# aehogan/lammps-induced-dipole-polarization-pair-style

Hardware: AMD Instinct MI355X
Metric: atom-steps/sec (higher is better)
Workload: dtype f64

## Files before the change

### lammps-induced-dipole-polarization-pair-style_amd/csrc/lab/api_env_knobs.inc

```
  if (const char *e = getenv("POLAR_ABLATE")) h->ablate = atoi(e);
  if (const char *e = getenv("POLAR_HOST_COLORS")) h->host_colors = atoi(e) != 0;
  if (const char *e = getenv("POLAR_SWEEP_KERNEL")) h->sweep_kernel = atoi(e);
  if (const char *e = getenv("POLAR_TILE_WAVES")) h->tile_waves = atoi(e) == 8 ? 8 : 4;
  if (const char *e = getenv("POLAR_TILE_WIDE")) h->tile_wide = atoi(e) != 0;
  if (const char *e = getenv("POLAR_CACHE_R2")) h->cache_r2 = atoi(e);
  if (const char *e = getenv("POLAR_LJ_TYPED")) h->lj_typed = atoi(e) != 0;
  if (const char *e = getenv("POLAR_STATIC_XQ")) h->static_xq = atoi(e) != 0;
  if (const char *e = getenv("POLAR_POL_FIRST")) h->pol_first = atoi(e) != 0;
  if (const char *e = getenv("POLAR_LP_WG_PER_CU")) h->lp_wg_per_cu = atoi(e);
  if (const char *e = getenv("POLAR_LP_QM")) h->lp_quad_major = atoi(e) != 0;
  if (const char *e = getenv("POLAR_LP_TILES")) h->lp_tiles = atoi(e) == 1 ? 1 : 2;
  if (const char *e = getenv("POLAR_LP_ROWS")) h->lp_rows = std::max(1, std::min(64, atoi(e)));
  if (const char *e = getenv("POLAR_LP_PAIRS")) h->lp_pairs = atoi(e) != 0;
  if (const char *e = getenv("POLAR_CLUSTER_DIST")) h->cluster_dist = atof(e);
  if (const char *e = getenv("POLAR_CLUSTER_MAX")) h->cluster_max = std::max(1, std::min(4, atoi(e)));
  if (const char *e = getenv("POLAR_LP_DEPTH")) { int v = atoi(e); h->lp_depth = (v == 2 || v == 3) ? v : 0; }
  if (const char *e = getenv("POLAR_QUAD_BLOCK")) { int v = atoi(e); if (v >= 64 && v <= 1024 && v % 64 == 0) h->quad_block = v; }
  if (const char *e = getenv("POLAR_FIELD_BLOCK")) { int v = atoi(e); if (v >= 64 && v <= 1024 && v % 64 == 0) h->field_block = v; }
```

### lammps-induced-dipole-polarization-pair-style_amd/csrc/polar_common.hpp

```cpp
#pragma once

#include <hip/hip_runtime.h>
#include <stdint.h>

#ifdef POLAR_LAB
#define POLAR_LAB_PARAM , int ablate
#define POLAR_LAB_PASS , ablate
#define POLAR_ABL(bit) (ablate & (bit))
#else
#define POLAR_LAB_PARAM
#define POLAR_LAB_PASS
#define POLAR_ABL(bit) 0
#endif

namespace polar {


struct __attribute__((aligned(64))) AtomRec {
  double x, mx;
  double y, my;
  double z, mz;
  double q, a;
};

// ... 227 lines not shown
  const double2 p0 = *reinterpret_cast<const double2 *>(base + ((j0 << 5) + piece));
  const double2 p1 = *reinterpret_cast<const double2 *>(base + ((j1 << 5) + piece));
  stage[h2 * 3 + k] = p0; stage[(32 + h2) * 3 + k] = p1;
  __builtin_amdgcn_fence(__ATOMIC_RELEASE, "wavefront");
  __builtin_amdgcn_wave_barrier();
  __builtin_amdgcn_fence(__ATOMIC_ACQUIRE, "wavefront");
  XQ r;
  r.a = stage[lane * 3]; r.b = stage[lane * 3 + 1];
  __builtin_amdgcn_wave_barrier();
  return r;
}

struct ExpCoef {
  double log2e, ln2hi, ln2lo;
  double c[14];
};
inline ExpCoef make_expcoef() {
  ExpCoef K;
  K.log2e = 1.4426950408889634074; K.ln2hi = 6.93147180369123816490e-01; K.ln2lo = 1.90821492927058770002e-10;
  const double c[14] = {1.0, 1.0, 0.5, 0.16666666666666666, 0.041666666666666664, 0.008333333333333333, 0.001388888888888889, 0.0001984126984126984, 2.48015873015873e-05, 2.7557319223985893e-06, 2.755731922398589e-07, 2.505210838544172e-08, 2.08767569878681e-09, 1.6059043836821613e-10};
  for (int k = 0; k < 14; k++) K.c[k] = c[k];
  return K;
}
__device__ __forceinline__ double exp_neg(double x, const ExpCoef &K) {
  x = fmax(x, -745.0);
  const double n = rint(x * K.log2e);
  double r = fma(-n, K.ln2hi, x);
  r = fma(-n, K.ln2lo, r);
  double p = K.c[13];
#pragma unroll
  for (int k = 12; k >= 0; k--) p = fma(p, r, K.c[k]);
  return ldexp(p, (int)n);
}

template <int DAMP>
__device__ __forceinline__ void tensor_scalars(double r2, double pd, double &s3, double &s5) {
  double rinv = rsqrt(r2);
  double r = r2 * rinv;
  double rinv2 = rinv * rinv;
  double r3 = rinv * rinv2;
  double r5 = r3 * rinv2;
  if (DAMP == 0) {
    double ar = pd * r;
    double e = exp(-ar);
    double p2 = 1.0 + ar + 0.5 * ar * ar;
    double p3 = p2 + ar * ar * ar * (1.0 / 6.0);
    s3 = (1.0 - e * p2) * r3;
    s5 = 3.0 * (1.0 - e * p3) * r5;
  } else {
    s3 = r3;
    s5 = 3.0 * r5;
  }
}
template <int DAMP>
__device__ __forceinline__ void tensor_scalars_k(double r2, double pd, const ExpCoef &K, double &s3, double &s5) {
  double rinv = rsqrt(r2);
  double r = r2 * rinv;
  double rinv2 = rinv * rinv;
  double r3 = rinv * rinv2;
  double r5 = r3 * rinv2;
  if (DAMP == 0) {
    double ar = pd * r;
    double e = exp_neg(-ar, K);
    double p2 = 1.0 + ar + 0.5 * ar * ar;
    double p3 = p2 + ar * ar * ar * (1.0 / 6.0);
    s3 = (1.0 - e * p2) * r3;
// ... 22 lines not shown
```

### lammps-induced-dipole-polarization-pair-style_amd/csrc/polar_handle.hpp

```cpp
#pragma once
#include <hip/hip_runtime.h>

#include <algorithm>
#include <initializer_list>
#include <utility>
#include <chrono>
#include <cmath>
#include <cstdio>
#include <cstdlib>
#include <exception>
#include <cstring>
#include <numeric>
#include <string>
#include <thread>
#include <mutex>
#include <condition_variable>
#include <functional>
#include <memory>
#include <stdexcept>
#include <unistd.h>
#include <vector>

#include "pair_host.hpp"
#include "polar_kernels.hpp"
// ... 165 lines not shown
  long long slots_epoch = -1;
  bool colors_recheck = false;
  std::vector<int> h_color;
  DBuf<int> d_color_orig, d_color_s;
  DBuf<int> d_klist;
  DBuf<int> d_cadj, d_cdeg, d_ccnt, d_cflags, d_crelabel;
  DBuf<unsigned long long> d_cprio;
  DBuf<double> d_cstat;
  DBuf<long long> d_coff;
  int *h_cflags = nullptr;
  double *h_cstat = nullptr;
  long long *h_coff = nullptr;
  int cadj_pitch = 16;
  int host_colors = 0;
  int colors_reused = 0, colors_rebuilt = 0;
  double ms_color_host = 0.0;
  double color_dist = 2.4;
  int field_block = 256;
  double bbox_lo[3] = {0, 0, 0}, bbox_hi[3] = {0, 0, 0};
  long long global_count = 0;
  DBuf<double> d_xchg; DBuf<int> d_xidx;
  bool device_list = false;
  int user_full_list = 0;
  long long lj_pitch = 0;
  DBuf<double4> d_ljpos; DBuf<int2> d_ljaux; DBuf<int> d_tag, d_nspecial, d_special, d_ljcell_id, d_ljcell_cnt, d_ljcell_fill; DBuf<long long> d_ljcell_first; DBuf<double> d_cutneighsq;
  int lj_typed = 1;
  bool lj_tab_arith = false;
  int lj_pers = 1;
  int ncu = 0;
  int lj_pers_threads = 768;
  bool sym_typed = false, dev_typed = false;
  int static_xq = 1;
  int pol_first = 1;
  int part_k = 0, part_n = 1;
  int lp_wg_per_cu = 0;
  int lp_quad_major = 1;
  int quad_block = POLAR_BLOCK;
  int lp_tiles = 2;
  int lp_rows = 1;
  int lp_pairs = 0;
  DBuf<int> d_ulead, d_udd_j;
  DBuf<long long> d_upos;
  DBuf<int2> d_unit;
  DBuf<int4> d_udesc;
  std::vector<int> unit_off;
  long long upitch = 0;
  int lp_depth = 0;
  int cache_r2 = -1;
  int stream_mode = 1;
  int sweep_kernel = 2;
  int ablate = 0;
  DBuf<SRec> d_srec0, d_srec1;
  DBuf<TileHdr> d_thdr;
  DBuf<TileRowEnt> d_trow;
  DBuf<int> d_un_j;
  DBuf<unsigned short> d_dd16;
  DBuf<double> d_pend;
  int un_pitch = 0;
  int un_lds = 0;
  long long pitch16 = 0;
  int tile_max_u = 0;
  bool tile_reported = false;
  double dens = 0.0;
  std::vector<TileLaunch> tile_launches;
  TileLaunch tile_all{};
  size_t tile_lds_attr[16] = {0, 0, 0, 0, 0, 0, 0, 0, 0, 0, 0, 0, 0, 0, 0, 0};
// ... 216 lines not shown
```

### lammps-induced-dipole-polarization-pair-style_amd/csrc/polar_rows.hpp

```cpp
#pragma once

#include "polar_common.hpp"

namespace polar {

static __global__ void k_pack(int n, const int *__restrict__ perm, const double *__restrict__ x, const double *__restrict__ q,
                       const double *__restrict__ alpha, const int *__restrict__ mol, const double *__restrict__ mu0,
                       AtomRec *__restrict__ r0, AtomRec *__restrict__ r1, int *__restrict__ mol_s,
                       double4 *__restrict__ pos4, double4 *__restrict__ xq_s, int wrap, Box box, double lo0, double lo1,
                       double lo2) {
  int i = blockIdx.x * blockDim.x + threadIdx.x;
  if (i == n) {
    AtomRec d;
    d.x = n > 0 ? x[0] : 0.0; d.y = n > 0 ? x[1] : 0.0; d.z = n > 0 ? x[2] : 0.0;
    d.mx = d.my = d.mz = d.q = d.a = 0.0;
    r0[n] = d; r1[n] = d;
  }
  if (i >= n) return;
  const int o = perm ? perm[i] : i;
  AtomRec r;
  r.x = x[3 * o]; r.y = x[3 * o + 1]; r.z = x[3 * o + 2]; r.q = q[o];
  if (wrap) {
    const double lo[3] = {lo0, lo1, lo2};
    double fr[3];
    frac_coords(box, lo, r.x, r.y, r.z, fr);
    const double n2 = box.periodic[2] ? floor(fr[2]) : 0.0, n1 = box.periodic[1] ? floor(fr[1]) : 0.0,
                 n0 = box.periodic[0] ? floor(fr[0]) : 0.0;
    r.z -= n2 * box.prd[2]; r.y -= n2 * box.yz + n1 * box.prd[1]; r.x -= n2 * box.xz + n1 * box.xy + n0 * box.prd[0];
  }
  r.mx = mu0 ? mu0[3 * o] : 0.0; r.my = mu0 ? mu0[3 * o + 1] : 0.0; r.mz = mu0 ? mu0[3 * o + 2] : 0.0;
  r.a = alpha[o];
  r0[i] = r;
  r1[i] = r;
  mol_s[i] = mol[o];
  if (pos4) pos4[i] = make_double4(r.x, r.y, r.z, __hiloint2double(mol[o], r.a != 0.0 ? 1 : 0));
// ... 413 lines not shown
      mx *= gamma; my *= gamma; mz *= gamma;
      rec0[i].mx = mx; rec0[i].my = my; rec0[i].mz = mz;
      rec1[i].mx = mx; rec1[i].my = my; rec1[i].mz = mz;
    }
  }
}

template <bool ALLPAIRS>
static __global__ __launch_bounds__(POLAR_BLOCK) void k_static_field(const int *__restrict__ rows, int nrows, int nlocal,
                                                              const AtomRec *__restrict__ rec,
                                                              const int *__restrict__ mol, Box box,
                                                              RowList nl,
                                                              const int *__restrict__ nl_j, double cut_coulsq,
                                                              double e2s, double gamma, int use_previous,
                                                              double *__restrict__ ef, AtomRec *__restrict__ rec0,
                                                              AtomRec *__restrict__ rec1, const double4 *__restrict__ xq_s) {
  static_field_body<ALLPAIRS, false>(rows, nrows, nlocal, rec, mol, box, nl, nl_j, cut_coulsq, e2s, gamma, use_previous, ef, rec0, rec1,
                                     xq_s, 0.0, nullptr);
}
template <bool ALLPAIRS>
static __global__ __launch_bounds__(POLAR_BLOCK) void k_ew_static_field(const int *__restrict__ rows, int nrows, int nlocal,
                                                                 const AtomRec *__restrict__ rec,
                                                                 const int *__restrict__ mol, Box box,
                                                                 RowList nl,
                                                                 const int *__restrict__ nl_j, double cut_coulsq,
                                                                 double e2s, double gamma, int use_previous,
                                                                 double *__restrict__ ef, AtomRec *__restrict__ rec0,
                                                                 AtomRec *__restrict__ rec1, const double4 *__restrict__ xq_s,
                                                                 double g_ewald, const double *__restrict__ erec) {
  static_field_body<ALLPAIRS, true>(rows, nrows, nlocal, rec, mol, box, nl, nl_j, cut_coulsq, e2s, gamma, use_previous, ef, rec0, rec1,
                                    xq_s, g_ewald, erec);
}

template <bool ALLPAIRS, int DAMP, bool EFLAG, bool VPAIR, bool EW>
static __device__ __forceinline__ void polar_force_body(const int *__restrict__ rows, int nrows, const int *__restrict__ perm,
                                                             int nlocal, const Scal *scal_in,
                                                             const AtomRec *__restrict__ recA,
                                                             const AtomRec *__restrict__ recB,
                                                             const int *__restrict__ mol, Box box,
                                                             RowList nl,
                                                             const int *__restrict__ nl_j, double cut_coulsq,
                                                             double ddcutsq, double pd, double e2s,
                                                             double *__restrict__ f, double *__restrict__ slots,
                                                             double *__restrict__ vatom, int vglobal, ExpCoef K,
                                                             double *__restrict__ dbg6, double g_ewald) {
  const int lane = threadIdx.x & 63;
  const int row = blockIdx.x * POLAR_ROWS_PER_BLOCK + (threadIdx.x >> 6);
  if (row >= nrows) return;
  const int i = rows ? rows[row] : row;
  const AtomRec *__restrict__ rec = __builtin_amdgcn_readfirstlane(scal_in->cur) ? recB : recA;
  const AtomRec ri = uniform_rec(rec[i]);
  const int mi = mol[i];
  const double f_shift = -1.0 / cut_coulsq;
  double fx = 0, fy = 0, fz = 0, uef = 0, udd = 0;
  double v0 = 0, v1 = 0, v2 = 0, v3 = 0, v4 = 0, v5 = 0;
  const bool isdbg = dbg6 && (perm ? perm[i] : i) == 0;
  double ddx = 0, ddy = 0, ddz = 0;
  long long beg = 0, end = nlocal;
  if (!ALLPAIRS) row_range(nl, i, beg, end);
  for (long long p = beg + lane; p < end; p += 64) {
    const int e = ALLPAIRS ? (int)p : nl_j[p];
    const int j = ALLPAIRS ? e : (e & POLAR_NL_MASK);
    if (j == i) continue;
    const AtomRec rj = *reinterpret_cast<const AtomRec *>(reinterpret_cast<const char *>(rec) + ((unsigned)j << 6));
    const bool molok = ALLPAIRS ? ((mi != mol[j]) || mi == 0) : !(e & POLAR_NL_SAMEMOL);
    double dx, dy, dz;
    pair_del<ALLPAIRS>(box, ri.x, ri.y, ri.z, rj.x, rj.y, rj.z, dx, dy, dz);
    const double xsq = dx * dx, ysq = dy * dy, zsq = dz * dz;
    const double rsq = xsq + ysq + zsq;
    const double rinv = rsqrt(rsq);
    const double r2inv = rinv * rinv;
    const double r = rsq * rinv;
    const double r3inv = r2inv * rinv;
    double px = 0, py = 0, pz = 0;
    if (EW) {
      if (rsq <= cut_coulsq) {
        double b1, b2;
        ewald_b12(rsq, g_ewald, molok, b1, b2);
        if (ri.a != 0.0 && rj.q != 0.0) {
          const double c = rj.q * e2s, pr = (ri.mx * dx + ri.my * dy + ri.mz * dz) * b2;
          px += c * (b1 * ri.mx - pr * dx); py += c * (b1 * ri.my - pr * dy); pz += c * (b1 * ri.mz - pr * dz);
        }
        if (rj.a != 0.0 && ri.q != 0.0) {
          const double c = ri.q * e2s, pr = (rj.mx * dx + rj.my * dy + rj.mz * dz) * b2;
          px -= c * (b1 * rj.mx - pr * dx); py -= c * (b1 * rj.my - pr * dy); pz -= c * (b1 * rj.mz - pr * dz);
        }
      }
    } else if (rsq < cut_coulsq && molok) {
      const double mxx = (-2.0 * xsq + ysq + zsq) * r2inv + f_shift * (ysq + zsq);
      const double myy = (-2.0 * ysq + xsq + zsq) * r2inv + f_shift * (xsq + zsq);
      const double mzz = (-2.0 * zsq + xsq + ysq) * r2inv + f_shift * (xsq + ysq);
      const double k = -(3.0 * r2inv + f_shift);
      const double mxy = k * dx * dy, mxz = k * dx * dz, myz = k * dy * dz;
      const double ef_temp = (r2inv + f_shift) * rinv * e2s;
      if (ri.a != 0.0 && rj.q != 0.0) {
        const double cf = rj.q * e2s * r3inv;
        px += cf * (ri.mx * mxx + ri.my * mxy + ri.mz * mxz);
        py += cf * (ri.mx * mxy + ri.my * myy + ri.mz * myz);
        pz += cf * (ri.mx * mxz + ri.my * myz + ri.mz * mzz);
        if (EFLAG) uef -= ef_temp * rj.q * (ri.mx * dx + ri.my * dy + ri.mz * dz);
      }
      if (rj.a != 0.0 && ri.q != 0.0) {
        const double cf = ri.q * e2s * r3inv;
        px -= cf * (rj.mx * mxx + rj.my * mxy + rj.mz * mxz);
        py -= cf * (rj.mx * mxy + rj.my * myy + rj.mz * myz);
        pz -= cf * (rj.mx * mxz + rj.my * myz + rj.mz * mzz);
        if (EFLAG) uef += ef_temp * ri.q * (rj.mx * dx + rj.my * dy + rj.mz * dz);
      }
    }
    if (ri.a != 0.0 && rj.a != 0.0 && (ALLPAIRS || rsq < ddcutsq)) {
      const double r5inv = r3inv * r2inv, r7inv = r5inv * r2inv;
      const double pdotp = ri.mx * rj.mx + ri.my * rj.my + ri.mz * rj.mz;
      const double pidotr = ri.mx * dx + ri.my * dy + ri.mz * dz;
      const double pjdotr = rj.mx * dx + rj.my * dy + rj.mz * dz;
      double pre_r, pre2, pre3;
      if (DAMP == 0) {
        const double t1 = exp_neg(-pd * r, K);
        const double t2 = 1.0 + pd * r + 0.5 * pd * pd * r * r;
        const double t3 = t2 + (1.0 / 6.0) * pd * pd * pd * r * r * r;
        const double g2 = 1.0 - t1 * t2, g3 = 1.0 - t1 * t3;
        const double pre1 = 3.0 * r5inv * pdotp * g2 - 15.0 * r7inv * pidotr * pjdotr * g3;
        pre2 = 3.0 * r5inv * pjdotr * g3;
        pre3 = 3.0 * r5inv * pidotr * g3;
        const double pre4 = -pdotp * r3inv * (-t1 * (pd * rinv + pd * pd) + t1 * pd * t2 * rinv);
        const double pre5 = 3.0 * pidotr * pjdotr * r5inv *
                            (-t1 * (pd * rinv + pd * pd + 0.5 * r * pd * pd * pd) + t1 * pd * t3 * rinv);
        pre_r = pre1 + pre4 + pre5;
        if (EFLAG) udd += r3inv * pdotp * g2 - 3.0 * r5inv * pidotr * pjdotr * g3;
      } else {
        pre_r = 3.0 * r5inv * pdotp - 15.0 * r7inv * pidotr * pjdotr;
        pre2 = 3.0 * r5inv * pjdotr;
        pre3 = 3.0 * r5inv * pidotr;
        if (EFLAG) udd += r3inv * pdotp - 3.0 * r5inv * pidotr * pjdotr;
      }
      const double qx = pre_r * dx + pre2 * ri.mx + pre3 * rj.mx, qy = pre_r * dy + pre2 * ri.my + pre3 * rj.my,
                   qz = pre_r * dz + pre2 * ri.mz + pre3 * rj.mz;
      px += qx; py += qy; pz += qz;
      if (isdbg) { ddx += qx; ddy += qy; ddz += qz; }
    }
    fx += px; fy += py; fz += pz;
    if (VPAIR) {
      v0 += 0.5 * dx * px; v1 += 0.5 * dy * py; v2 += 0.5 * dz * pz;
      v3 += 0.5 * dx * py; v4 += 0.5 * dx * pz; v5 += 0.5 * dy * pz;
    }
  }
  fx = wave_sum(fx); fy = wave_sum(fy); fz = wave_sum(fz);
  if (lane == 0) {
    const int o = perm ? perm[i] : i;
    atomicAdd(&f[3 * o], fx); atomicAdd(&f[3 * o + 1], fy); atomicAdd(&f[3 * o + 2], fz);
  }
  if (isdbg) {
    ddx = wave_sum(ddx); ddy = wave_sum(ddy); ddz = wave_sum(ddz);
    if (lane == 0) { dbg6[0] = fx; dbg6[1] = fy; dbg6[2] = fz; dbg6[3] = ddx; dbg6[4] = ddy; dbg6[5] = ddz; }
  }
  if (EFLAG) {
    uef = wave_sum(uef); udd = wave_sum(udd);
    if (lane == 0) {
      if (ri.a != 0.0) atomicAdd(slot_ptr(slots, SL_USELF), 0.5 * (ri.mx * ri.mx + ri.my * ri.my + ri.mz * ri.mz) / ri.a);
      atomicAdd(slot_ptr(slots, SL_UEF), 0.5 * uef);
      atomicAdd(slot_ptr(slots, SL_UDD), 0.5 * udd);
    }
  }
  if (VPAIR) {
    v0 = wave_sum(v0); v1 = wave_sum(v1); v2 = wave_sum(v2); v3 = wave_sum(v3); v4 = wave_sum(v4); v5 = wave_sum(v5);
    if (lane == 0) {
      if (vglobal) {
        atomicAdd(slot_ptr(slots, SL_V0), v0); atomicAdd(slot_ptr(slots, SL_V1), v1); atomicAdd(slot_ptr(slots, SL_V2), v2);
        atomicAdd(slot_ptr(slots, SL_V3), v3); atomicAdd(slot_ptr(slots, SL_V4), v4); atomicAdd(slot_ptr(slots, SL_V5), v5);
      }
      if (vatom) {
        double *va = vatom + 6 * (size_t)(perm ? perm[i] : i);
        va[0] += v0; va[1] += v1; va[2] += v2; va[3] += v3; va[4] += v4; va[5] += v5;
      }
    }
  }
}

template <bool ALLPAIRS, int DAMP, bool EFLAG, bool VPAIR>
static __global__ __launch_bounds__(POLAR_BLOCK) void k_polar_force(
    const int *__restrict__ rows, int nrows, const int *__restrict__ perm, int nlocal, const Scal *scal_in,
    const AtomRec *__restrict__ recA, const AtomRec *__restrict__ recB, const int *__restrict__ mol, Box box, RowList nl,
    const int *__restrict__ nl_j, double cut_coulsq, double ddcutsq, double pd, double e2s, double *__restrict__ f,
    double *__restrict__ slots, double *__restrict__ vatom, int vglobal, ExpCoef K, double *__restrict__ dbg6) {
  polar_force_body<ALLPAIRS, DAMP, EFLAG, VPAIR, false>(rows, nrows, perm, nlocal, scal_in, recA, recB, mol, box, nl, nl_j, cut_coulsq, ddcutsq, pd, e2s, f, slots, vatom, vglobal, K, dbg6, 0.0);
}
template <bool ALLPAIRS, int DAMP, bool EFLAG, bool VPAIR>
static __global__ __launch_bounds__(POLAR_BLOCK) void k_ew_polar_force(
    const int *__restrict__ rows, int nrows, const int *__restrict__ perm, int nlocal, const Scal *scal_in,
    const AtomRec *__restrict__ recA, const AtomRec *__restrict__ recB, const int *__restrict__ mol, Box box, RowList nl,
    const int *__restrict__ nl_j, double cut_coulsq, double ddcutsq, double pd, double e2s, double *__restrict__ f,
    double *__restrict__ slots, double *__restrict__ vatom, int vglobal, ExpCoef K, double *__restrict__ dbg6, double g_ewald) {
  polar_force_body<ALLPAIRS, DAMP, EFLAG, VPAIR, true>(rows, nrows, perm, nlocal, scal_in, recA, recB, mol, box, nl, nl_j, cut_coulsq, ddcutsq, pd, e2s, f, slots, vatom, vglobal, K, dbg6, g_ewald);
}

static __global__ void k_add_into(long long n, const double *__restrict__ src, double *__restrict__ dst) {
  long long i = blockIdx.x * (long long)blockDim.x + threadIdx.x;
  if (i < n) dst[i] += src[i];
}

static __global__ __launch_bounds__(POLAR_BLOCK) void k_virial_fdotr(int nall, const double *__restrict__ x,
                                                              const double *__restrict__ f, double *__restrict__ slots) {
  double v[6] = {0, 0, 0, 0, 0, 0};
  for (int i = blockIdx.x * blockDim.x + threadIdx.x; i < nall; i += gridDim.x * blockDim.x) {
    const double fx = f[3 * i], fy = f[3 * i + 1], fz = f[3 * i + 2];
    const double xx = x[3 * i], yy = x[3 * i + 1], zz = x[3 * i + 2];
    v[0] += fx * xx; v[1] += fy * yy; v[2] += fz * zz; v[3] += fy * xx; v[4] += fz * xx; v[5] += fz * yy;
  }
  const int lane = threadIdx.x & 63;
#pragma unroll
  for (int k = 0; k < 6; k++) {
    double s = wave_sum(v[k]);
    if (lane == 0 && s != 0.0) atomicAdd(slot_ptr(slots, SL_V0 + k), s);
  }
}

}
```

### lammps-induced-dipole-polarization-pair-style_amd/csrc/polar_solver.hpp

```cpp
#pragma once

#include "polar_common.hpp"

namespace polar {

enum { EP_JACOBI = 0, EP_INPLACE = 1, EP_FIELD = 2 };

template <bool ALLPAIRS, int DAMP, int EP>
static __global__ __launch_bounds__(1024) void k_field(int nrows, const int *__restrict__ rows, int nlocal,
                                                       AtomRec *__restrict__ recA, AtomRec *__restrict__ recB, Box box,
                                                       RowList ddl,
                                                       const int *__restrict__ dd_j,
                                                       const double2 *__restrict__ dd_s, double ddcutsq, double pd,
                                                       const double *__restrict__ ef, double *__restrict__ Fout,
                                                       const Scal *scal, double *__restrict__ slots POLAR_LAB_PARAM) {
  if (scal->done) return;
  const int lane = threadIdx.x & 63;
  const int row = blockIdx.x * (blockDim.x >> 6) + (threadIdx.x >> 6);
  if (row >= nrows) return;
  const int i = rows ? rows[row] : row;
  const int cur = scal->cur;
  const AtomRec *__restrict__ src = (EP == EP_JACOBI && cur) ? recB : recA;
  AtomRec *__restrict__ dst = (EP == EP_JACOBI) ? (cur ? recA : recB) : recA;
  const AtomRec ri = src[i];
// ... 19 lines not shown
      }
    } else {
#ifdef POLAR_LAB
#include "lab/sweep_register_staged_body.hpp"
#endif
    }
    if (ALLPAIRS) { fx = wave_sum(fx); fy = wave_sum(fy); fz = wave_sum(fz); }
  }
  if (lane == 0) {
    if (EP == EP_FIELD) {
      Fout[3 * i] = fx; Fout[3 * i + 1] = fy; Fout[3 * i + 2] = fz;
    } else {
      const double a = ri.a;
      const double mx = a * (ef[3 * i] + fx), my = a * (ef[3 * i + 1] + fy), mz = a * (ef[3 * i + 2] + fz);
      const double ddx = mx - ri.mx, ddy = my - ri.my, ddz = mz - ri.mz;
      dst[i].mx = mx; dst[i].my = my; dst[i].mz = mz;
      const double c = ddx * ddx + ddy * ddy + ddz * ddz;
      if (c != 0.0 && !POLAR_ABL(16)) atomicAdd(slot_ptr(slots, SL_CHANGE), c);
    }
  }
}

#ifdef POLAR_LAB
#include "lab/sweep_quad.hpp"
#endif

template <int R>
__device__ __forceinline__ void lp_gather(const char *srcc, int joff, unsigned piece, char *tile) {
  const unsigned o_ = (unsigned)__builtin_amdgcn_update_dpp(0, joff, R * 0x55, 0xF, 0xF, true) + piece;
  const char *g = srcc + o_;
  __builtin_amdgcn_global_load_lds((const __attribute__((address_space(1))) void *)g,
                                   (__attribute__((address_space(3))) void *)(tile + R * 1024), 16, 0, 0);
}
__device__ __forceinline__ double rsqrt_pos(double x) {
  const double y = __builtin_amdgcn_rsq(x);
  const double e = fma(-(x * y), y, 1.0);
  return fma(y * e, 0.5, y);
}
__device__ __forceinline__ double exp_neg_fast(double x, const ExpCoef &K) {
  x = fmax(x, -700.0);
  const double shift = 6755399441055744.0;
  const double ns = fma(x, K.log2e, shift);
  const double n = ns - shift;
  double r = fma(-n, K.ln2hi, x);
  r = fma(-n, K.ln2lo, r);
  double p = K.c[10];
#pragma unroll
  for (int k = 9; k >= 0; k--) p = fma(p, r, K.c[k]);
  return __hiloint2double(__double2hiint(p) + (__double2loint(ns) << 20), __double2loint(p));
}
template <int DAMP>
__device__ __forceinline__ void tensor_scalars_lp(double r2, double pd, const ExpCoef &K, double &s3, double &s5) {
  const double rinv = rsqrt_pos(r2);
  const double rinv2 = rinv * rinv;
  const double r3 = rinv * rinv2;
  const double r5 = r3 * rinv2;
  if (DAMP == 0) {
    const double ar = pd * (r2 * rinv);
    const double e = exp_neg_fast(-ar, K);
    const double ar2 = ar * ar;
    const double p2 = fma(ar2, 0.5, 1.0 + ar);
    const double p3 = fma(ar2 * ar, 1.0 / 6.0, p2);
    s3 = fma(-e, p2, 1.0) * r3;
    s5 = fma(-e, p3, 1.0) * (3.0 * r5);
  } else {
    s3 = r3;
    s5 = 3.0 * r5;
  }
}
struct LpSelf { double mu_old, alpha, ef; };
__device__ __forceinline__ LpSelf lp_self(int lane, const AtomRec *self, const double *efi) {
  LpSelf s{0.0, 0.0, 0.0};
  if (lane < 3) {
    const double *r = reinterpret_cast<const double *>(self);
    s.mu_old = r[2 * lane + 1]; s.alpha = r[7]; s.ef = efi[lane];
  }
  return s;
}
template <bool DET>
__device__ __forceinline__ void lp_finish(double ax, double ay, double az, int lane, const LpSelf &self, AtomRec *out,
                                          double *slots, double omega, double *pend) {
  const bool odd = lane & 1, hi = lane & 2;
  const double keep1 = odd ? ay : ax, give1 = odd ? ax : ay;
// ... 304 lines not shown
```

### lammps-induced-dipole-polarization-pair-style_amd/csrc/polar_step.hip

```cpp
#include "polar_handle.hpp"

void launch_scan(long long n, const int *in, long long *out, DBuf<long long> &tot, hipStream_t s) {
  const int nb = (int)std::max<long long>(1, (n + POLAR_SCAN_ITEMS - 1) / POLAR_SCAN_ITEMS);
  tot.ensure((size_t)nb + 1);
  k_scan_block<<<nb, 1024, 0, s>>>(n, in, out, tot.p);
  if (nb > 1) {
    k_scan_totals<<<1, 1024, 0, s>>>(nb, tot.p, out + n);
    k_scan_add<<<nblk(n - POLAR_SCAN_ITEMS, 256), 256, 0, s>>>(n, out, tot.p);
  }
}

void build_cells(polar_handle *h) {
  const polar_settings &st = h->ph.st;
  const int n = h->nlocal;
  const double cutall = std::max(st.cut_coul, st.dd_cutoff);
  double width[3];
  box_widths(h->box, width);
  for (int k = 0; k < 3; k++)
    if (h->box.periodic[k] && width[k] < 2.0 * cutall * (1.0 - 1e-12))
      throw InputError("dd_cutoff mode needs box lengths >= 2*max(cut_coul,dd_cutoff); use exact mode (dd_cutoff 0)");
  CellGrid &g = h->grid;
  g.trim = 1;
#ifdef POLAR_LAB
  if (const char *e = getenv("POLAR_NL_TRIM")) g.trim = atoi(e);
// ... 321 lines not shown
    launch_field_dyn<EP_JACOBI>(h, ap, own_n(h), own_rows(h));
    return;
  }
  const int ncol = (int)h->color_off.size() - 1;
  for (int c = 0; c < ncol; c++) {
    const int cnt = h->color_off[c + 1] - h->color_off[c];
    if (cnt <= 0) continue;
    launch_field_dyn<EP_INPLACE>(h, false, cnt, h->d_rows.p + h->color_off[c]);
  }
}

void sweep_phase(polar_handle *h, int c, int part) {
  const int ncol = (int)h->color_off.size() - 1;
  if (c < 0 || c >= ncol) throw std::logic_error("sweep_phase: no such colour");
  const int a = h->color_off[c], b = h->color_off[c + 1];
  const int m = (h->color_nsub == 2 && !deterministic(h)) ? h->color_sub[2 * c + 1] : b;
  const int lo = part == 2 ? m : a, hi = part == 1 ? m : b;
  launch_field_lp<EP_INPLACE>(h, hi - lo, h->d_lpdesc.p + lo);
}
template <bool AP, int DAMP>
void launch_force(polar_handle *h, int eflag, int vglobal, double *vatom, double *fdst) {
  const bool vpair = vglobal || vatom;
  const polar_settings &st = h->ph.st;
  dim3 grid(nblk(own_n(h), POLAR_ROWS_PER_BLOCK)), block(POLAR_BLOCK);
  const double ccs = st.cut_coul * st.cut_coul, dds = st.dd_cutoff * st.dd_cutoff, e2s = std::sqrt(h->P.qqrd2e);
  double *dbg6 = nullptr;
  if (st.debug) {
    h->d_dbgf.ensure(8);
    HIPCHECK(hipMemsetAsync(h->d_dbgf.p, 0, 8 * sizeof(double), h->stream));
    dbg6 = h->d_dbgf.p;
  }
  const bool ew = ewald_on(h);
  const double g = h->P.g_ewald;
#define LF(E, V)                                                                                                    \
  if (ew) k_ew_polar_force<AP, DAMP, E, V><<<grid, block, 0, h->stream>>>(own_rows(h), own_n(h), h->sorted ? h->d_perm.p : nullptr, h->nlocal, h->d_scal.p, h->d_rec0.p, h->d_rec1.p,  \
                                                               h->d_mol_s.p, h->box, RowList{h->d_nl_cnt.p, h->nl_pitch}, h->d_nl_j.p,  \
                                                               ccs, dds, st.polar_damp, e2s, fdst, h->d_slots.p, vatom, vglobal, make_expcoef(),  \
                                                               dbg6, g);                                        \
  else k_polar_force<AP, DAMP, E, V><<<grid, block, 0, h->stream>>>(own_rows(h), own_n(h), h->sorted ? h->d_perm.p : nullptr, h->nlocal, h->d_scal.p, h->d_rec0.p, h->d_rec1.p,  \
                                                               h->d_mol_s.p, h->box, RowList{h->d_nl_cnt.p, h->nl_pitch}, h->d_nl_j.p,  \
                                                               ccs, dds, st.polar_damp, e2s, fdst, h->d_slots.p, vatom, vglobal, make_expcoef(),  \
                                                               dbg6)
  if (eflag) { if (vpair) { LF(true, true); } else { LF(true, false); } }
  else       { if (vpair) { LF(false, true); } else { LF(false, false); } }
#undef LF
}

size_t ewald_lds_per_atom(int nm) { return 3 * (size_t)(nm + 1) * sizeof(double2) + 3 * sizeof(double); }
int ewald_tile(int nm) { return (int)std::max<size_t>(1, std::min<size_t>(32, (48 * 1024) / ewald_lds_per_atom(nm))); }

void ewald_kvectors(polar_handle *h) {
  const Box &b = h->box;
  const double g = h->P.g_ewald, acc = h->ph.st.polar_ewald;
  std::vector<double> key = {b.prd[0], b.prd[1], b.prd[2], b.xy, b.xz, b.yz, g, acc};
  if (key == h->ew_key) return;
  const double lx = b.prd[0], ly = b.prd[1], lz = b.prd[2], xy = b.xy, xz = b.xz, yz = b.yz;
  const double i00 = 1.0 / lx, i01 = -xy / (lx * ly), i02 = (xy * yz - ly * xz) / (lx * ly * lz), i11 = 1.0 / ly,
               i12 = -yz / (ly * lz), i22 = 1.0 / lz;
  const double vol = lx * ly * lz, twopi = 2.0 * M_PI;
  const double kcut = 2.0 * g * std::sqrt(-std::log(acc)), kcut2 = kcut * kcut;
  const int hm = (int)std::floor(kcut * lx / twopi), km = (int)std::floor(kcut * std::sqrt(xy * xy + ly * ly) / twopi),
            lm = (int)std::floor(kcut * std::sqrt(xz * xz + yz * yz + lz * lz) / twopi);
  std::vector<double4> kv;
  std::vector<int4> hkl, rows;
  for (int ih = 0; ih <= hm; ih++)
    for (int ik = (ih == 0 ? 0 : -km); ik <= km; ik++) {
      int row = -1;
      for (int il = (ih == 0 && ik == 0 ? 1 : -lm); il <= lm; il++) {
        const double kx = twopi * (ih * i00), ky = twopi * (ih * i01 + ik * i11), kz = twopi * (ih * i02 + ik * i12 + il * i22);
        const double k2 = kx * kx + ky * ky + kz * kz;
        if (k2 > kcut2 || k2 == 0.0) continue;
        if (row < 0) { row = (int)rows.size(); rows.push_back(make_int4(ih, ik, il, (int)kv.size())); }
        kv.push_back(make_double4(kx, ky, kz, 8.0 * M_PI / vol * std::exp(-k2 / (4.0 * g * g)) / k2));
        hkl.push_back(make_int4(ih, ik, il, 0));
      }
    }
  h->ew_nk = (int)kv.size();
  h->ew_nrow = (int)rows.size();
// ... 636 lines not shown
```

Before: 15.56 million.

## Refactor polar force pair into reduced-arithmetic helper with prefetched neighbor records

Result: faster. 15.89 million, median of 6 (+2.1%).

```diff
diff --git a/lammps-induced-dipole-polarization-pair-style_amd/csrc/lab/api_env_knobs.inc b/lammps-induced-dipole-polarization-pair-style_amd/csrc/lab/api_env_knobs.inc
--- a/lammps-induced-dipole-polarization-pair-style_amd/csrc/lab/api_env_knobs.inc
+++ b/lammps-induced-dipole-polarization-pair-style_amd/csrc/lab/api_env_knobs.inc
@@ -17,3 +17,4 @@
   if (const char *e = getenv("POLAR_LP_DEPTH")) { int v = atoi(e); h->lp_depth = (v == 2 || v == 3) ? v : 0; }
   if (const char *e = getenv("POLAR_QUAD_BLOCK")) { int v = atoi(e); if (v >= 64 && v <= 1024 && v % 64 == 0) h->quad_block = v; }
   if (const char *e = getenv("POLAR_FIELD_BLOCK")) { int v = atoi(e); if (v >= 64 && v <= 1024 && v % 64 == 0) h->field_block = v; }
+  if (const char *e = getenv("POLAR_FORCE_LITERAL")) h->force_literal = atoi(e) != 0;
diff --git a/lammps-induced-dipole-polarization-pair-style_amd/csrc/lab/force_pair_literal.hpp b/lammps-induced-dipole-polarization-pair-style_amd/csrc/lab/force_pair_literal.hpp
--- /dev/null
+++ b/lammps-induced-dipole-polarization-pair-style_amd/csrc/lab/force_pair_literal.hpp
@@ -0,0 +1,84 @@
+#pragma once
+
+namespace polar {
+
+template <bool ALLPAIRS, int DAMP, bool EFLAG, bool EW>
+__device__ __forceinline__ void polar_force_pair_literal(const ExpCoef &K, double g_ewald, double dx, double dy, double dz,
+                                                         const AtomRec &ri, const AtomRec &rj, bool molok, double cut_coulsq,
+                                                         double ddcutsq, double pd, double e2s, double &px, double &py,
+                                                         double &pz, double &ddx, double &ddy, double &ddz, double &uef,
+                                                         double &udd) {
+  const double f_shift = -1.0 / cut_coulsq;
+  const double xsq = dx * dx, ysq = dy * dy, zsq = dz * dz;
+  const double rsq = xsq + ysq + zsq;
+  const double rinv = rsqrt(rsq);
+  const double r2inv = rinv * rinv;
+  const double r = rsq * rinv;
+  const double r3inv = r2inv * rinv;
+  px = 0; py = 0; pz = 0; ddx = 0; ddy = 0; ddz = 0; uef = 0; udd = 0;
+  if (EW) {
+    if (rsq <= cut_coulsq) {
+      double b1, b2;
+      ewald_b12(rsq, g_ewald, molok, b1, b2);
+      if (ri.a != 0.0 && rj.q != 0.0) {
+        const double c = rj.q * e2s, pr = (ri.mx * dx + ri.my * dy + ri.mz * dz) * b2;
+        px += c * (b1 * ri.mx - pr * dx); py += c * (b1 * ri.my - pr * dy); pz += c * (b1 * ri.mz - pr * dz);
+      }
+      if (rj.a != 0.0 && ri.q != 0.0) {
+        const double c = ri.q * e2s, pr = (rj.mx * dx + rj.my * dy + rj.mz * dz) * b2;
+        px -= c * (b1 * rj.mx - pr * dx); py -= c * (b1 * rj.my - pr * dy); pz -= c * (b1 * rj.mz - pr * dz);
+      }
+    }
+  } else if (rsq < cut_coulsq && molok) {
+    const double mxx = (-2.0 * xsq + ysq + zsq) * r2inv + f_shift * (ysq + zsq);
+    const double myy = (-2.0 * ysq + xsq + zsq) * r2inv + f_shift * (xsq + zsq);
+    const double mzz = (-2.0 * zsq + xsq + ysq) * r2inv + f_shift * (xsq + ysq);
+    const double k = -(3.0 * r2inv + f_shift);
+    const double mxy = k * dx * dy, mxz = k * dx * dz, myz = k * dy * dz;
+    const double ef_temp = (r2inv + f_shift) * rinv * e2s;
+    if (ri.a != 0.0 && rj.q != 0.0) {
+      const double cf = rj.q * e2s * r3inv;
+      px += cf * (ri.mx * mxx + ri.my * mxy + ri.mz * mxz);
+      py += cf * (ri.mx * mxy + ri.my * myy + ri.mz * myz);
+      pz += cf * (ri.mx * mxz + ri.my * myz + ri.mz * mzz);
+      if (EFLAG) uef -= ef_temp * rj.q * (ri.mx * dx + ri.my * dy + ri.mz * dz);
+    }
+    if (rj.a != 0.0 && ri.q != 0.0) {
+      const double cf = ri.q * e2s * r3inv;
+      px -= cf * (rj.mx * mxx + rj.my * mxy + rj.mz * mxz);
+      py -= cf * (rj.mx * mxy + rj.my * myy + rj.mz * myz);
+      pz -= cf * (rj.mx * mxz + rj.my * myz + rj.mz * mzz);
+      if (EFLAG) uef += ef_temp * ri.q * (rj.mx * dx + rj.my * dy + rj.mz * dz);
+    }
+  }
+  if (ri.a != 0.0 && rj.a != 0.0 && (ALLPAIRS || rsq < ddcutsq)) {
+    const double r5inv = r3inv * r2inv, r7inv = r5inv * r2inv;
+    const double pdotp = ri.mx * rj.mx + ri.my * rj.my + ri.mz * rj.mz;
+    const double pidotr = ri.mx * dx + ri.my * dy + ri.mz * dz;
+    const double pjdotr = rj.mx * dx + rj.my * dy + rj.mz * dz;
+    double pre_r, pre2, pre3;
+    if (DAMP == 0) {
+      const double t1 = exp_neg(-pd * r, K);
+      const double t2 = 1.0 + pd * r + 0.5 * pd * pd * r * r;
+      const double t3 = t2 + (1.0 / 6.0) * pd * pd * pd * r * r * r;
+      const double g2 = 1.0 - t1 * t2, g3 = 1.0 - t1 * t3;
+      const double pre1 = 3.0 * r5inv * pdotp * g2 - 15.0 * r7inv * pidotr * pjdotr * g3;
+      pre2 = 3.0 * r5inv * pjdotr * g3;
+      pre3 = 3.0 * r5inv * pidotr * g3;
+      const double pre4 = -pdotp * r3inv * (-t1 * (pd * rinv + pd * pd) + t1 * pd * t2 * rinv);
+      const double pre5 = 3.0 * pidotr * pjdotr * r5inv *
+                          (-t1 * (pd * rinv + pd * pd + 0.5 * r * pd * pd * pd) + t1 * pd * t3 * rinv);
+      pre_r = pre1 + pre4 + pre5;
+      if (EFLAG) udd += r3inv * pdotp * g2 - 3.0 * r5inv * pidotr * pjdotr * g3;
+    } else {
+      pre_r = 3.0 * r5inv * pdotp - 15.0 * r7inv * pidotr * pjdotr;
+      pre2 = 3.0 * r5inv * pjdotr;
+      pre3 = 3.0 * r5inv * pidotr;
+      if (EFLAG) udd += r3inv * pdotp - 3.0 * r5inv * pidotr * pjdotr;
+    }
+    ddx = pre_r * dx + pre2 * ri.mx + pre3 * rj.mx; ddy = pre_r * dy + pre2 * ri.my + pre3 * rj.my;
+    ddz = pre_r * dz + pre2 * ri.mz + pre3 * rj.mz;
+  }
+}
+
+}
diff --git a/lammps-induced-dipole-polarization-pair-style_amd/csrc/polar_common.hpp b/lammps-induced-dipole-polarization-pair-style_amd/csrc/polar_common.hpp
--- a/lammps-induced-dipole-polarization-pair-style_amd/csrc/polar_common.hpp
+++ b/lammps-induced-dipole-polarization-pair-style_amd/csrc/polar_common.hpp
@@ -283,6 +283,30 @@
   for (int k = 12; k >= 0; k--) p = fma(p, r, K.c[k]);
   return ldexp(p, (int)n);
 }
+__device__ __forceinline__ double rsqrt_pos(double x) {
+  const double y = __builtin_amdgcn_rsq(x);
+  const double e = fma(-(x * y), y, 1.0);
+  return fma(y * e, 0.5, y);
+}
+__device__ __forceinline__ double rsqrt_pos3(double x) {
+  const double y = __builtin_amdgcn_rsq(x);
+  const double e = fma(-(x * y), y, 1.0);
+  return fma(y * e, fma(e, 0.375, 0.5), y);
+}
+template <int DEG = 10>
+__device__ __forceinline__ double exp_neg_fast(double x, const ExpCoef &K) {
+  static_assert(DEG >= 1 && DEG <= 13, "ExpCoef holds 1/k! up to k = 13");
+  x = fmax(x, -700.0);
+  const double shift = 6755399441055744.0;
+  const double ns = fma(x, K.log2e, shift);
+  const double n = ns - shift;
+  double r = fma(-n, K.ln2hi, x);
+  r = fma(-n, K.ln2lo, r);
+  double p = K.c[DEG];
+#pragma unroll
+  for (int k = DEG - 1; k >= 0; k--) p = fma(p, r, K.c[k]);
+  return __hiloint2double(__double2hiint(p) + (__double2loint(ns) << 20), __double2loint(p));
+}
 
 template <int DAMP>
 __device__ __forceinline__ void tensor_scalars(double r2, double pd, double &s3, double &s5) {
diff --git a/lammps-induced-dipole-polarization-pair-style_amd/csrc/polar_force_pair.hpp b/lammps-induced-dipole-polarization-pair-style_amd/csrc/polar_force_pair.hpp
--- /dev/null
+++ b/lammps-induced-dipole-polarization-pair-style_amd/csrc/polar_force_pair.hpp
@@ -0,0 +1,97 @@
+#pragma once
+
+#if defined(__HIPCC__)
+#define POLAR_PAIR_FN __host__ __device__ __forceinline__
+#else
+#define POLAR_PAIR_FN inline
+#endif
+
+namespace polar {
+
+struct PairRow {
+  double mx, my, mz;
+  double wx, wy, wz;
+  double eq;
+  bool pol;
+};
+POLAR_PAIR_FN PairRow make_pair_row(double mx, double my, double mz, double q, double alpha, double e2s) {
+  PairRow r;
+  r.pol = alpha != 0.0;
+  r.mx = r.pol ? mx : 0.0; r.my = r.pol ? my : 0.0; r.mz = r.pol ? mz : 0.0;
+  r.wx = e2s * r.mx; r.wy = e2s * r.my; r.wz = e2s * r.mz;
+  r.eq = e2s * q;
+  return r;
+}
+
+struct PairCut {
+  double cut_coulsq;
+  double ddcutsq;
+  double f_shift;
+  double pd;
+};
+
+template <bool ALLPAIRS, int DAMP, bool EFLAG, bool EW, bool WANT_P, class M>
+POLAR_PAIR_FN void polar_force_pair(const M &m, double dx, double dy, double dz, const PairRow &ri, double mjx, double mjy,
+                                    double mjz, double qj, double aj, bool molok, const PairCut &c, double &cdx, double &cdy,
+                                    double &cdz, double &ddx, double &ddy, double &ddz, double &uef, double &udd, double &px,
+                                    double &py, double &pz) {
+  const double rsq = dx * dx + dy * dy + dz * dz;
+  const double rinv = m.rsqrt(rsq);
+  const double r2inv = rinv * rinv;
+  const double r3inv = r2inv * rinv;
+  const bool polj = aj != 0.0;
+  if (WANT_P) { px = 0.0; py = 0.0; pz = 0.0; }
+  if (EW ? (rsq <= c.cut_coulsq) : (rsq < c.cut_coulsq && molok)) {
+    const double eqi = polj ? ri.eq : 0.0;
+    const double wx = qj * ri.wx - eqi * mjx, wy = qj * ri.wy - eqi * mjy, wz = qj * ri.wz - eqi * mjz;
+    const double wd = wx * dx + wy * dy + wz * dz;
+    double ca, cb;
+    if (EW) {
+      m.ewald_b12(rsq, molok, ca, cb);
+    } else {
+      ca = (1.0 + c.f_shift * rsq) * r3inv;
+      cb = (3.0 * r2inv + c.f_shift) * r3inv;
+      if (EFLAG) uef -= ((r2inv + c.f_shift) * rinv) * wd;
+    }
+    const double t = cb * wd;
+    const double cx = ca * wx - t * dx, cy = ca * wy - t * dy, cz = ca * wz - t * dz;
+    cdx += cx; cdy += cy; cdz += cz;
+    if (WANT_P) { px = cx; py = cy; pz = cz; }
+  }
+  if (ri.pol && polj && (ALLPAIRS || rsq < c.ddcutsq)) {
+    const double r5inv = r3inv * r2inv;
+    const double pdotp = ri.mx * mjx + ri.my * mjy + ri.mz * mjz;
+    const double pidotr = ri.mx * dx + ri.my * dy + ri.mz * dz;
+    const double pjdotr = mjx * dx + mjy * dy + mjz * dz;
+    const double pipj = pidotr * pjdotr;
+    double cpp, cdd, s5, u3;
+    if (DAMP == 0) {
+      const double a = c.pd * (rsq * rinv);
+      const double t = m.exp_neg(-a);
+      const double a2 = a * a, a3 = a2 * a;
+      const double p2 = 1.0 + a + 0.5 * a2;
+      const double ta3 = t * a3;
+      const double g2 = 1.0 - t * p2;
+      const double g3 = g2 - (1.0 / 6.0) * ta3;
+      s5 = 3.0 * r5inv * g3;
+      cpp = r5inv * (3.0 * g2 - 0.5 * ta3);
+      cdd = (r5inv * r2inv) * (0.5 * (ta3 * a) - 15.0 * g3);
+      u3 = r3inv * g2;
+    } else {
+      s5 = 3.0 * r5inv;
+      cpp = s5;
+      cdd = -5.0 * (s5 * r2inv);
+      u3 = r3inv;
+    }
+    const double pre_r = cpp * pdotp + cdd * pipj;
+    const double pre2 = s5 * pjdotr, pre3 = s5 * pidotr;
+    const double qx = pre_r * dx + pre2 * ri.mx + pre3 * mjx;
+    const double qy = pre_r * dy + pre2 * ri.my + pre3 * mjy;
+    const double qz = pre_r * dz + pre2 * ri.mz + pre3 * mjz;
+    ddx += qx; ddy += qy; ddz += qz;
+    if (WANT_P) { px += qx; py += qy; pz += qz; }
+    if (EFLAG) udd += u3 * pdotp - s5 * pipj;
+  }
+}
+
+}
diff --git a/lammps-induced-dipole-polarization-pair-style_amd/csrc/polar_handle.hpp b/lammps-induced-dipole-polarization-pair-style_amd/csrc/polar_handle.hpp
--- a/lammps-induced-dipole-polarization-pair-style_amd/csrc/polar_handle.hpp
+++ b/lammps-induced-dipole-polarization-pair-style_amd/csrc/polar_handle.hpp
@@ -221,6 +221,9 @@
   bool sym_typed = false, dev_typed = false;
   int static_xq = 1;
   int pol_first = 1;
+#ifdef POLAR_LAB
+  int force_literal = 0;
+#endif
   int part_k = 0, part_n = 1;
   int lp_wg_per_cu = 0;
   int lp_quad_major = 1;
diff --git a/lammps-induced-dipole-polarization-pair-style_amd/csrc/polar_rows.hpp b/lammps-induced-dipole-polarization-pair-style_amd/csrc/polar_rows.hpp
--- a/lammps-induced-dipole-polarization-pair-style_amd/csrc/polar_rows.hpp
+++ b/lammps-induced-dipole-polarization-pair-style_amd/csrc/polar_rows.hpp
@@ -1,6 +1,15 @@
 #pragma once
 
 #include "polar_common.hpp"
+#include "polar_force_pair.hpp"
+#ifdef POLAR_LAB
+#include "lab/force_pair_literal.hpp"
+#define POLAR_LIT_PARAM , int literal
+#define POLAR_LIT_PASS , literal
+#else
+#define POLAR_LIT_PARAM
+#define POLAR_LIT_PASS
+#endif
 
 namespace polar {
 
@@ -480,6 +489,14 @@
                                     xq_s, g_ewald, erec);
 }
 
+struct PairMath {
+  const ExpCoef &K;
+  double g_ewald;
+  __device__ __forceinline__ double rsqrt(double x) const { return rsqrt_pos3(x); }
+  __device__ __forceinline__ double exp_neg(double x) const { return exp_neg_fast<12>(x, K); }
+  __device__ __forceinline__ void ewald_b12(double rsq, bool kept, double &b1, double &b2) const { polar::ewald_b12(rsq, g_ewald, kept, b1, b2); }
+};
+
 template <bool ALLPAIRS, int DAMP, bool EFLAG, bool VPAIR, bool EW>
 static __device__ __forceinline__ void polar_force_body(const int *__restrict__ rows, int nrows, const int *__restrict__ perm,
                                                              int nlocal, const Scal *scal_in,
@@ -491,7 +508,7 @@
                                                              double ddcutsq, double pd, double e2s,
                                                              double *__restrict__ f, double *__restrict__ slots,
                                                              double *__restrict__ vatom, int vglobal, ExpCoef K,
-                                                             double *__restrict__ dbg6, double g_ewald) {
+                                                             double *__restrict__ dbg6, double g_ewald POLAR_LIT_PARAM) {
   const int lane = threadIdx.x & 63;
   const int row = blockIdx.x * POLAR_ROWS_PER_BLOCK + (threadIdx.x >> 6);
   if (row >= nrows) return;
@@ -499,99 +516,59 @@
   const AtomRec *__restrict__ rec = __builtin_amdgcn_readfirstlane(scal_in->cur) ? recB : recA;
   const AtomRec ri = uniform_rec(rec[i]);
   const int mi = mol[i];
-  const double f_shift = -1.0 / cut_coulsq;
+  const PairRow pri = make_pair_row(ri.mx, ri.my, ri.mz, ri.q, ri.a, e2s);
+  const PairCut cut{cut_coulsq, ddcutsq, -1.0 / cut_coulsq, pd};
+  const PairMath pm{K, g_ewald};
   double fx = 0, fy = 0, fz = 0, uef = 0, udd = 0;
   double v0 = 0, v1 = 0, v2 = 0, v3 = 0, v4 = 0, v5 = 0;
   const bool isdbg = dbg6 && (perm ? perm[i] : i) == 0;
   double ddx = 0, ddy = 0, ddz = 0;
   long long beg = 0, end = nlocal;
   if (!ALLPAIRS) row_range(nl, i, beg, end);
+  Box pbox = box;
+  if (!ALLPAIRS) {
+#pragma unroll
+    for (int k = 0; k < 3; k++) { pbox.inv[k] = box.periodic[k] ? box.inv[k] : 0.0; pbox.periodic[k] = 1; }
+  }
+  int e_n1 = i, e_n2 = i;
+  if (!ALLPAIRS) {
+    if (beg + lane < end) e_n1 = nl_j[beg + lane];
+    if (beg + lane + 64 < end) e_n2 = nl_j[beg + lane + 64];
+  }
+  AtomRec r_n1 = rec[e_n1 & POLAR_NL_MASK];
   for (long long p = beg + lane; p < end; p += 64) {
-    const int e = ALLPAIRS ? (int)p : nl_j[p];
+    const int e = ALLPAIRS ? (int)p : e_n1;
     const int j = ALLPAIRS ? e : (e & POLAR_NL_MASK);
+    const AtomRec rj = ALLPAIRS ? rec[j] : r_n1;
+    if (!ALLPAIRS) {
+      e_n1 = e_n2;
+      r_n1 = *reinterpret_cast<const AtomRec *>(reinterpret_cast<const char *>(rec) + ((unsigned)(e_n1 & POLAR_NL_MASK) << 6));
+      e_n2 = p + 128 < end ? nl_j[p + 128] : i;
+    }
     if (j == i) continue;
-    const AtomRec rj = *reinterpret_cast<const AtomRec *>(reinterpret_cast<const char *>(rec) + ((unsigned)j << 6));
     const bool molok = ALLPAIRS ? ((mi != mol[j]) || mi == 0) : !(e & POLAR_NL_SAMEMOL);
     double dx, dy, dz;
-    pair_del<ALLPAIRS>(box, ri.x, ri.y, ri.z, rj.x, rj.y, rj.z, dx, dy, dz);
-    const double xsq = dx * dx, ysq = dy * dy, zsq = dz * dz;
-    const double rsq = xsq + ysq + zsq;
-    const double rinv = rsqrt(rsq);
-    const double r2inv = rinv * rinv;
-    const double r = rsq * rinv;
-    const double r3inv = r2inv * rinv;
-    double px = 0, py = 0, pz = 0;
-    if (EW) {
-      if (rsq <= cut_coulsq) {
-        double b1, b2;
-        ewald_b12(rsq, g_ewald, molok, b1, b2);
-        if (ri.a != 0.0 && rj.q != 0.0) {
-          const double c = rj.q * e2s, pr = (ri.mx * dx + ri.my * dy + ri.mz * dz) * b2;
-          px += c * (b1 * ri.mx - pr * dx); py += c * (b1 * ri.my - pr * dy); pz += c * (b1 * ri.mz - pr * dz);
-        }
-        if (rj.a != 0.0 && ri.q != 0.0) {
-          const double c = ri.q * e2s, pr = (rj.mx * dx + rj.my * dy + rj.mz * dz) * b2;
-          px -= c * (b1 * rj.mx - pr * dx); py -= c * (b1 * rj.my - pr * dy); pz -= c * (b1 * rj.mz - pr * dz);
-        }
-      }
-    } else if (rsq < cut_coulsq && molok) {
-      const double mxx = (-2.0 * xsq + ysq + zsq) * r2inv + f_shift * (ysq + zsq);
-      const double myy = (-2.0 * ysq + xsq + zsq) * r2inv + f_shift * (xsq + zsq);
-      const double mzz = (-2.0 * zsq + xsq + ysq) * r2inv + f_shift * (xsq + ysq);
-      const double k = -(3.0 * r2inv + f_shift);
-      const double mxy = k * dx * dy, mxz = k * dx * dz, myz = k * dy * dz;
-      const double ef_temp = (r2inv + f_shift) * rinv * e2s;
-      if (ri.a != 0.0 && rj.q != 0.0) {
-        const double cf = rj.q * e2s * r3inv;
-        px += cf * (ri.mx * mxx + ri.my * mxy + ri.mz * mxz);
-        py += cf * (ri.mx * mxy + ri.my * myy + ri.mz * myz);
-        pz += cf * (ri.mx * mxz + ri.my * myz + ri.mz * mzz);
-        if (EFLAG) uef -= ef_temp * rj.q * (ri.mx * dx + ri.my * dy + ri.mz * dz);
-      }
-      if (rj.a != 0.0 && ri.q != 0.0) {
-        const double cf = ri.q * e2s * r3inv;
-        px -= cf * (rj.mx * mxx + rj.my * mxy + rj.mz * mxz);
-        py -= cf * (rj.mx * mxy + rj.my * myy + rj.mz * myz);
-        pz -= cf * (rj.mx * mxz + rj.my * myz + rj.mz * mzz);
-        if (EFLAG) uef += ef_temp * ri.q * (rj.mx * dx + rj.my * dy + rj.mz * dz);
-      }
-    }
-    if (ri.a != 0.0 && rj.a != 0.0 && (ALLPAIRS || rsq < ddcutsq)) {
-      const double r5inv = r3inv * r2inv, r7inv = r5inv * r2inv;
-      const double pdotp = ri.mx * rj.mx + ri.my * rj.my + ri.mz * rj.mz;
-      const double pidotr = ri.mx * dx + ri.my * dy + ri.mz * dz;
-      const double pjdotr = rj.mx * dx + rj.my * dy + rj.mz * dz;
-      double pre_r, pre2, pre3;
-      if (DAMP == 0) {
-        const double t1 = exp_neg(-pd * r, K);
-        const double t2 = 1.0 + pd * r + 0.5 * pd * pd * r * r;
-        const double t3 = t2 + (1.0 / 6.0) * pd * pd * pd * r * r * r;
-        const double g2 = 1.0 - t1 * t2, g3 = 1.0 - t1 * t3;
-        const double pre1 = 3.0 * r5inv * pdotp * g2 - 15.0 * r7inv * pidotr * pjdotr * g3;
-        pre2 = 3.0 * r5inv * pjdotr * g3;
-        pre3 = 3.0 * r5inv * pidotr * g3;
-        const double pre4 = -pdotp * r3inv * (-t1 * (pd * rinv + pd * pd) + t1 * pd * t2 * rinv);
-        const double pre5 = 3.0 * pidotr * pjdotr * r5inv *
-                            (-t1 * (pd * rinv + pd * pd + 0.5 * r * pd * pd * pd) + t1 * pd * t3 * rinv);
-        pre_r = pre1 + pre4 + pre5;
-        if (EFLAG) udd += r3inv * pdotp * g2 - 3.0 * r5inv * pidotr * pjdotr * g3;
-      } else {
-        pre_r = 3.0 * r5inv * pdotp - 15.0 * r7inv * pidotr * pjdotr;
-        pre2 = 3.0 * r5inv * pjdotr;
-        pre3 = 3.0 * r5inv * pidotr;
-        if (EFLAG) udd += r3inv * pdotp - 3.0 * r5inv * pidotr * pjdotr;
-      }
-      const double qx = pre_r * dx + pre2 * ri.mx + pre3 * rj.mx, qy = pre_r * dy + pre2 * ri.my + pre3 * rj.my,
-                   qz = pre_r * dz + pre2 * ri.mz + pre3 * rj.mz;
-      px += qx; py += qy; pz += qz;
-      if (isdbg) { ddx += qx; ddy += qy; ddz += qz; }
-    }
-    fx += px; fy += py; fz += pz;
+    pair_del<ALLPAIRS>(pbox, ri.x, ri.y, ri.z, rj.x, rj.y, rj.z, dx, dy, dz);
+    double px, py, pz;
+#ifdef POLAR_LAB
+    if (literal) {
+      double qx, qy, qz, ue, ud;
+      polar_force_pair_literal<ALLPAIRS, DAMP, EFLAG, EW>(K, g_ewald, dx, dy, dz, ri, rj, molok, cut_coulsq, ddcutsq, pd, e2s, px, py, pz,
+                                                          qx, qy, qz, ue, ud);
+      fx += px; fy += py; fz += pz;
+      ddx += qx; ddy += qy; ddz += qz;
+      if (VPAIR) { px += qx; py += qy; pz += qz; }
+      if (EFLAG) { uef += ue; udd += ud; }
+    } else
+#endif
+    polar_force_pair<ALLPAIRS, DAMP, EFLAG, EW, VPAIR>(pm, dx, dy, dz, pri, rj.mx, rj.my, rj.mz, rj.q, rj.a, molok, cut, fx, fy, fz,
+                                                       ddx, ddy, ddz, uef, udd, px, py, pz);
     if (VPAIR) {
       v0 += 0.5 * dx * px; v1 += 0.5 * dy * py; v2 += 0.5 * dz * pz;
       v3 += 0.5 * dx * py; v4 += 0.5 * dx * pz; v5 += 0.5 * dy * pz;
     }
   }
+  fx += ddx; fy += ddy; fz += ddz;
   fx = wave_sum(fx); fy = wave_sum(fy); fz = wave_sum(fz);
   if (lane == 0) {
     const int o = perm ? perm[i] : i;
@@ -629,16 +606,16 @@
     const int *__restrict__ rows, int nrows, const int *__restrict__ perm, int nlocal, const Scal *scal_in,
     const AtomRec *__restrict__ recA, const AtomRec *__restrict__ recB, const int *__restrict__ mol, Box box, RowList nl,
     const int *__restrict__ nl_j, double cut_coulsq, double ddcutsq, double pd, double e2s, double *__restrict__ f,
-    double *__restrict__ slots, double *__restrict__ vatom, int vglobal, ExpCoef K, double *__restrict__ dbg6) {
-  polar_force_body<ALLPAIRS, DAMP, EFLAG, VPAIR, false>(rows, nrows, perm, nlocal, scal_in, recA, recB, mol, box, nl, nl_j, cut_coulsq, ddcutsq, pd, e2s, f, slots, vatom, vglobal, K, dbg6, 0.0);
+    double *__restrict__ slots, double *__restrict__ vatom, int vglobal, ExpCoef K, double *__restrict__ dbg6 POLAR_LIT_PARAM) {
+  polar_force_body<ALLPAIRS, DAMP, EFLAG, VPAIR, false>(rows, nrows, perm, nlocal, scal_in, recA, recB, mol, box, nl, nl_j, cut_coulsq, ddcutsq, pd, e2s, f, slots, vatom, vglobal, K, dbg6, 0.0 POLAR_LIT_PASS);
 }
 template <bool ALLPAIRS, int DAMP, bool EFLAG, bool VPAIR>
 static __global__ __launch_bounds__(POLAR_BLOCK) void k_ew_polar_force(
     const int *__restrict__ rows, int nrows, const int *__restrict__ perm, int nlocal, const Scal *scal_in,
     const AtomRec *__restrict__ recA, const AtomRec *__restrict__ recB, const int *__restrict__ mol, Box box, RowList nl,
     const int *__restrict__ nl_j, double cut_coulsq, double ddcutsq, double pd, double e2s, double *__restrict__ f,
-    double *__restrict__ slots, double *__restrict__ vatom, int vglobal, ExpCoef K, double *__restrict__ dbg6, double g_ewald) {
-  polar_force_body<ALLPAIRS, DAMP, EFLAG, VPAIR, true>(rows, nrows, perm, nlocal, scal_in, recA, recB, mol, box, nl, nl_j, cut_coulsq, ddcutsq, pd, e2s, f, slots, vatom, vglobal, K, dbg6, g_ewald);
+    double *__restrict__ slots, double *__restrict__ vatom, int vglobal, ExpCoef K, double *__restrict__ dbg6, double g_ewald POLAR_LIT_PARAM) {
+  polar_force_body<ALLPAIRS, DAMP, EFLAG, VPAIR, true>(rows, nrows, perm, nlocal, scal_in, recA, recB, mol, box, nl, nl_j, cut_coulsq, ddcutsq, pd, e2s, f, slots, vatom, vglobal, K, dbg6, g_ewald POLAR_LIT_PASS);
 }
 
 static __global__ void k_add_into(long long n, const double *__restrict__ src, double *__restrict__ dst) {
@@ -663,3 +640,6 @@
 }
 
 }
+
+#undef POLAR_LIT_PARAM
+#undef POLAR_LIT_PASS
diff --git a/lammps-induced-dipole-polarization-pair-style_amd/csrc/polar_solver.hpp b/lammps-induced-dipole-polarization-pair-style_amd/csrc/polar_solver.hpp
--- a/lammps-induced-dipole-polarization-pair-style_amd/csrc/polar_solver.hpp
+++ b/lammps-induced-dipole-polarization-pair-style_amd/csrc/polar_solver.hpp
@@ -75,23 +75,6 @@
   __builtin_amdgcn_global_load_lds((const __attribute__((address_space(1))) void *)g,
                                    (__attribute__((address_space(3))) void *)(tile + R * 1024), 16, 0, 0);
 }
-__device__ __forceinline__ double rsqrt_pos(double x) {
-  const double y = __builtin_amdgcn_rsq(x);
-  const double e = fma(-(x * y), y, 1.0);
-  return fma(y * e, 0.5, y);
-}
-__device__ __forceinline__ double exp_neg_fast(double x, const ExpCoef &K) {
-  x = fmax(x, -700.0);
-  const double shift = 6755399441055744.0;
-  const double ns = fma(x, K.log2e, shift);
-  const double n = ns - shift;
-  double r = fma(-n, K.ln2hi, x);
-  r = fma(-n, K.ln2lo, r);
-  double p = K.c[10];
-#pragma unroll
-  for (int k = 9; k >= 0; k--) p = fma(p, r, K.c[k]);
-  return __hiloint2double(__double2hiint(p) + (__double2loint(ns) << 20), __double2loint(p));
-}
 template <int DAMP>
 __device__ __forceinline__ void tensor_scalars_lp(double r2, double pd, const ExpCoef &K, double &s3, double &s5) {
   const double rinv = rsqrt_pos(r2);
diff --git a/lammps-induced-dipole-polarization-pair-style_amd/csrc/polar_step.hip b/lammps-induced-dipole-polarization-pair-style_amd/csrc/polar_step.hip
--- a/lammps-induced-dipole-polarization-pair-style_amd/csrc/polar_step.hip
+++ b/lammps-induced-dipole-polarization-pair-style_amd/csrc/polar_step.hip
@@ -377,18 +377,24 @@
   }
   const bool ew = ewald_on(h);
   const double g = h->P.g_ewald;
+#ifdef POLAR_LAB
+#define POLAR_LIT_ARG , h->force_literal
+#else
+#define POLAR_LIT_ARG
+#endif
 #define LF(E, V)                                                                                                    \
   if (ew) k_ew_polar_force<AP, DAMP, E, V><<<grid, block, 0, h->stream>>>(own_rows(h), own_n(h), h->sorted ? h->d_perm.p : nullptr, h->nlocal, h->d_scal.p, h->d_rec0.p, h->d_rec1.p,  \
                                                                h->d_mol_s.p, h->box, RowList{h->d_nl_cnt.p, h->nl_pitch}, h->d_nl_j.p,  \
                                                                ccs, dds, st.polar_damp, e2s, fdst, h->d_slots.p, vatom, vglobal, make_expcoef(),  \
-                                                               dbg6, g);                                        \
+                                                               dbg6, g POLAR_LIT_ARG);                          \
   else k_polar_force<AP, DAMP, E, V><<<grid, block, 0, h->stream>>>(own_rows(h), own_n(h), h->sorted ? h->d_perm.p : nullptr, h->nlocal, h->d_scal.p, h->d_rec0.p, h->d_rec1.p,  \
                                                                h->d_mol_s.p, h->box, RowList{h->d_nl_cnt.p, h->nl_pitch}, h->d_nl_j.p,  \
                                                                ccs, dds, st.polar_damp, e2s, fdst, h->d_slots.p, vatom, vglobal, make_expcoef(),  \
-                                                               dbg6)
+                                                               dbg6 POLAR_LIT_ARG)
   if (eflag) { if (vpair) { LF(true, true); } else { LF(true, false); } }
   else       { if (vpair) { LF(false, true); } else { LF(false, false); } }
 #undef LF
+#undef POLAR_LIT_ARG
 }
 
 size_t ewald_lds_per_atom(int nm) { return 3 * (size_t)(nm + 1) * sizeof(double2) + 3 * sizeof(double); }
```
